# hzxie/Stereo-3D-Reconstruction

Hardware: NVIDIA B200
Metric: stereo pairs/sec Stereo2Voxel fwd (higher is better)
Workload: dtype bf16

## Files before the change

### include/s3d.h

```cpp
#ifndef S3D_H_
#define S3D_H_

#include <stdint.h>

#ifdef __cplusplus
extern "C" {
#endif

#define S3D_OK                0
#define S3D_ERR_INVALID      -1
#define S3D_ERR_CUDA         -2
#define S3D_ERR_UNSUPPORTED  -3

#define S3D_DTYPE_F32   0
#define S3D_DTYPE_BF16  1
#define S3D_DTYPE_BF16X2 2

#define S3D_ACT_NONE     0
#define S3D_ACT_RELU     1
#define S3D_ACT_LEAKY    2
#define S3D_ACT_SIGMOID  3
#define S3D_ACT_TANH     4

#define S3D_MAX_TAPS 64
// ... 33 lines not shown
                    const void* residual, void* out, void* stream);

int s3d_conv2d_halo(const void* in, const void* w, const float* bias, const void* residual, void* out, int nimg, int h, int wd,
                    int cin, int cout, int64_t osN, int64_t osH, int64_t osW, int relu, void* stream);

int s3d_pack_image(const float* img, const float* disp, float disp_scale, void* out,
                   int B, int H, int W, int Cpad, int out_dtype, void* stream);

int s3d_pack_image_u8(const uint8_t* img, const float* disp, float disp_scale, float img_scale, void* out,
                      int B, int H, int W, int Cpad, int out_dtype, void* stream);

int s3d_conv_first(const void* img, int img_u8, const float* disp, float disp_scale, const void* w, const float* bias,
                   void* out, int B, int H, int W, int cin, int cin_pad, int cout_pad, int dtype, int act,
                   float act_param, void* stream);

int s3d_conv_concat_volume(const S3dConvParams* p, const void* feat, int feat_pitch, int feat_pad, const float* bias,
                           void* out, void* stream);
int s3d_conv_concat_volume_ro(const S3dConvParams* p, const void* feat, int feat_pitch, int feat_pad, const void* w_refonce,
                              const float* bias, void* out, void* stream);
int s3d_concat_gonce_assemble(const float* maps_l, const float* maps_r, const float* edge_l, const float* edge_r,
                              const float* bias, void* out, int B, int D, int h, int w, int map_w, int out_dtype, void* stream);
int s3d_map_conv(const void* in, const void* w, float* out, int nimg, int h, int in_w, int ow, int off, int ntx, int cout,
                 int dtype, void* stream);
int s3d_cost_volume_concat(const void* feat, void* vol, int B, int h, int w, int C, int D,
                           int dtype, void* stream);
int s3d_soft_argmin(const float* cost, float* disp, int N, int D, int h, int w, float sign,
                    void* stream);


int s3d_tap_gather_soft_argmin(const float* taps, float* disp, float* disp_std_q, float* cost_out, int N, int D, int h, int w,
                               int tap_stride, float sign, void* stream);
int s3d_cls_soft_argmin(const void* x, const void* w_taps, float* disp, float* disp_std_q, int N, int D, int h, int w, int C,
                        float sign, void* stream);
int64_t s3d_conv_cls_workspace_bytes(int N, int D, int h, int w);
int s3d_conv_cls_soft_argmin(const S3dConvParams* p, const void* in, const float* bias, const void* w_taps, void* workspace,
                             float* disp, float* disp_std_q, float sign, void* stream);
int s3d_corr_soft_argmin(const void* feat, float* disp, float* disp_std_q, float* cost_out, int B, int h, int w,
                         int C, int c_real, int D, int dtype, void* stream);
int s3d_upsample_disp(const float* disp_q, float* disp, int N, int h, int w, int H, int W,
                      float scale, void* stream);
int s3d_upsample_disp_eval(const float* disp_q, float* disp, int B, int h, int w, int H, int W, float scale,
                           const float* gt, const float* thresholds, int T, float max_gt, long long* disp_stats,
                           uint8_t* lr_mask, float lr_thresh, long long* lr_stats,
                           const float* disp_std_q, float* disp_std, const float* unc_thresh, int K, long long* unc_stats,
                           void* stream);

// ... 36 lines not shown
```

### stereo_3d_reconstruction_b200/csrc/map_conv.cu

```cuda
#include <cuda.h>
#include <string.h>
#include "common.cuh"
#include "ptx.cuh"
#include "epilogue.cuh"

namespace s3d {
namespace {

constexpr int kThreads = 384;
constexpr int kTY = 16, kTX = 8;
constexpr int kMaxSlots = 6;
constexpr int kTapBytes = 8192;

struct McArgs {
  float* out;
  int nimg, h, ow, cout;
  int off;
  int ntx, ntaps, pitch;
  int patch_tx;
  int patch_bytes;
  int slots, nchunks;
  int tiles_x, tiles_per_img, total_tiles;
  uint32_t idesc;
};

struct McCtrl {
  uint64_t w_full, w_empty;
  uint64_t p_full[kMaxSlots], p_empty[kMaxSlots];
  uint64_t acc_full[2], acc_empty[2];
  uint32_t tmem_base;
};

template <int NTX, bool kSplit>
__global__ void __launch_bounds__(kThreads, 1)
map_conv_kernel(const __grid_constant__ CUtensorMap map_x, const __grid_constant__ CUtensorMap map_w, const __grid_constant__ McArgs a) {
  constexpr int kRowB = kSplit ? 128 : 64;
  constexpr int kNC = kSplit ? 64 : 128;
  constexpr uint64_t kLayout = kSplit ? 2ull : 4ull;
  static_assert(kNC * kRowB == kTapBytes, "tap bytes");
  extern __shared__ uint8_t smem_raw[];
  uint8_t* smem = reinterpret_cast<uint8_t*>((reinterpret_cast<uintptr_t>(smem_raw) + 1023) & ~uintptr_t(1023));
  uint8_t* smem_w = smem;
  uint8_t* smem_p = smem + a.ntaps * kTapBytes;
  __shared__ McCtrl ctrl;
  const int warp = threadIdx.x >> 5, lane = threadIdx.x & 31;

// ... 20 lines not shown
        for (int t0 = 0; t0 < a.ntaps; t0 += a.ntx)
          ptx::tma_load_3d(smem_w + t0 * kTapBytes, &map_w, &ctrl.w_full, 0, ch * kNC, t0);
        wphase ^= 1;
        for (int k = 0; k < my_tiles; ++k) {
          const int t = blockIdx.x + k * gridDim.x;
          const int img = t / a.tiles_per_img, r = t % a.tiles_per_img;
          const int y0 = (r / a.tiles_x) * kTY, j0 = (r % a.tiles_x) * kTX;
          ptx::mbar_wait(&ctrl.p_empty[slot], pphase ^ 1);
          ptx::mbar_arrive_expect_tx(&ctrl.p_full[slot], a.patch_tx);
          ptx::tma_load_5d(smem_p + slot * a.patch_bytes, &map_x, &ctrl.p_full[slot], 0, j0 + a.off, y0 - 1, 0, img);
          if (++slot == a.slots) { slot = 0; pphase ^= 1; }
        }
      }
    }
  } else if (warp == 1) {
    int slot = 0;  uint32_t pphase = 0, wphase = 0, aphase = 0;
    int buf = 0;
    const uint64_t hi_a = (static_cast<uint64_t>((a.pitch * kRowB) >> 4) << 32) | (1ull << 46) | (kLayout << 61);
    const uint64_t hi_b = (static_cast<uint64_t>((8 * kRowB) >> 4) << 32) | (1ull << 46) | (kLayout << 61);
    const uint32_t w_u = ptx::smem_u32(smem_w), p_u = ptx::smem_u32(smem_p);
    for (int ch = 0; ch < a.nchunks; ++ch) {
      ptx::mbar_wait(&ctrl.w_full, wphase);
      wphase ^= 1;
      for (int k = 0; k < my_tiles; ++k) {
        ptx::mbar_wait(&ctrl.acc_empty[buf], aphase ^ 1);
        ptx::mbar_wait(&ctrl.p_full[slot], pphase);
        ptx::tc_fence_after();
        const uint32_t pa = p_u + slot * a.patch_bytes, d_tmem = tmem_base + buf * kNC;
        const uint64_t ad0 = hi_a | ((pa >> 4) | (1u << 16)), bd0 = hi_b | ((w_u >> 4) | (1u << 16));
        if (ptx::elect_one()) {
#pragma unroll
          for (int t = 0; t < 3 * NTX; ++t) {
            constexpr int kPitch = kTX + NTX - 1;
            const uint64_t ad = ad0 + (uint64_t)((((t / NTX) * kPitch + (t % NTX)) * kRowB) >> 4);
            const uint64_t bd = bd0 + (uint64_t)((t * kTapBytes) >> 4);
            ptx::mma_bf16(d_tmem, ad, bd, a.idesc, t != 0);
            ptx::mma_bf16(d_tmem, ad + 2, bd + 2, a.idesc, 1u);
            if constexpr (kSplit) {
              ptx::mma_bf16(d_tmem, ad + 4, bd, a.idesc, 1u);      ptx::mma_bf16(d_tmem, ad + 6, bd + 2, a.idesc, 1u);
              ptx::mma_bf16(d_tmem, ad, bd + 4, a.idesc, 1u);      ptx::mma_bf16(d_tmem, ad + 2, bd + 6, a.idesc, 1u);
            }
          }
          ptx::tc_commit(&ctrl.p_empty[slot]);
          ptx::tc_commit(&ctrl.acc_full[buf]);
          if (k == my_tiles - 1) ptx::tc_commit(&ctrl.w_empty);
        }
        __syncwarp();
        if (++slot == a.slots) { slot = 0; pphase ^= 1; }
        if (++buf == 2) { buf = 0; aphase ^= 1; }
      }
      if (my_tiles == 0 && ptx::elect_one()) ptx::mbar_arrive(&ctrl.w_empty);
      __syncwarp();
    }
  } else if (warp >= 4) {
    const int q = warp & 3, grp = (warp - 4) >> 2;
    const int m = q * 32 + lane, yy = m >> 3, xx = m & 7;
    uint32_t aphase = 0;
    const int items = a.nchunks * my_tiles;
    for (int it = grp; it < items; it += 2) {
      const int ch = it / my_tiles, k = it % my_tiles;
      const int t = blockIdx.x + k * gridDim.x;
      const int img = t / a.tiles_per_img, r = t % a.tiles_per_img;
      const int y = (r / a.tiles_x) * kTY + yy, jt = (r % a.tiles_x) * kTX;
      float* op = a.out + (((int64_t)img * a.h + y) * a.ow + jt) * a.cout + ch * kNC + xx * 4;
      ptx::mbar_wait(&ctrl.acc_full[grp], aphase);
      ptx::tc_fence_after();
      const uint32_t taddr = tmem_base + grp * kNC + (static_cast<uint32_t>(q * 32) << 16);
#pragma unroll
      for (int half = 0; half < kNC / 64; ++half) {
        uint32_t v[4][16];
#pragma unroll
        for (int g = 0; g < 4; ++g) ptx::tmem_ld16(taddr + half * 64 + g * 16, v[g]);
        ptx::tmem_ld_wait();
        if (half == kNC / 64 - 1) {
          ptx::tc_fence_before();
          ptx::mbar_arrive(&ctrl.acc_empty[grp]);
        }
#pragma unroll
        for (int blk = 0; blk < 2; ++blk) {
          uint4 c[8];
#pragma unroll
          for (int i = 0; i < 8; ++i) {
            const uint32_t* src = &v[2 * blk + (i >> 2)][4 * (i & 3)];
            c[i] = make_uint4(src[0], src[1], src[2], src[3]);
          }
#pragma unroll
          for (int st = 4; st >= 1; st >>= 1) {
            const bool up = (lane & st) != 0;
#pragma unroll
            for (int i = 0; i < 8; ++i) {
              if (i & st) continue;
              const uint4 send = up ? c[i] : c[i | st];
              uint4 recv;
              recv.x = __shfl_xor_sync(0xffffffffu, send.x, st);  recv.y = __shfl_xor_sync(0xffffffffu, send.y, st);
              recv.z = __shfl_xor_sync(0xffffffffu, send.z, st);  recv.w = __shfl_xor_sync(0xffffffffu, send.w, st);
              if (up) c[i] = recv; else c[i | st] = recv;
            }
          }
          if (y < a.h) {
#pragma unroll
            for (int i = 0; i < 8; ++i)
              if (jt + i < a.ow) *reinterpret_cast<uint4*>(op + (int64_t)i * a.cout + half * 64 + blk * 32) = c[i];
          }
        }
      }
      aphase ^= 1;
    }
  }

  ptx::tc_fence_before();
  __syncthreads();
  if (warp == 2) {
    ptx::tc_fence_after();
    ptx::tmem_dealloc(tmem_base, 2 * kNC);
  }
}

}
}

extern "C" int s3d_map_conv(const void* in, const void* w, float* out, int nimg, int h, int in_w, int ow, int off, int ntx,
                            int cout, int dtype, void* stream) {
  using namespace s3d;
  if (!in || !w || !out) { set_error("map_conv: null argument"); return S3D_ERR_INVALID; }
  S3D_CHECK_ARG(dtype == S3D_DTYPE_BF16 || dtype == S3D_DTYPE_BF16X2, "map_conv: dtype %d (bf16 or the bf16 pair)", dtype);
  const bool split = dtype == S3D_DTYPE_BF16X2;
  const int kNC = split ? 64 : 128, kRowB = split ? 128 : 64;
  S3D_CHECK_ARG(nimg > 0 && h > 0 && ow > 0 && in_w > 0 && (ntx == 3 || ntx == 5) && cout > 0 && cout % 128 == 0,
                "map_conv: nimg=%d h=%d ow=%d in_w=%d ntx=%d cout=%d (ntx 3 or 5, cout a multiple of 128)", nimg, h, ow, in_w, ntx, cout);
  S3D_CHECK_ARG(off >= 0 && off + ow + ntx - 1 <= in_w + 8, "map_conv: output columns reach beyond the input rows");
  S3D_CHECK_ARG(((reinterpret_cast<uintptr_t>(in) | reinterpret_cast<uintptr_t>(w) | reinterpret_cast<uintptr_t>(out)) & 15) == 0,
                "map_conv: pointers must be 16-byte aligned");
  McArgs a;
  memset(&a, 0, sizeof(a));
  a.out = out;  a.nimg = nimg;  a.h = h;  a.ow = ow;  a.cout = cout;  a.off = off;
  a.ntx = ntx;  a.ntaps = 3 * ntx;  a.pitch = kTX + ntx - 1;
  a.patch_tx = (kTY + 2) * a.pitch * kRowB;
  a.patch_bytes = (a.patch_tx + 1023) / 1024 * 1024;
  a.nchunks = cout / kNC;
  a.tiles_x = ceil_div(ow, kTX);
  a.tiles_per_img = a.tiles_x * ceil_div(h, kTY);
  const int64_t total = (int64_t)nimg * a.tiles_per_img;
  S3D_CHECK_ARG(total < (1ll << 30), "map_conv: too many tiles");
  a.total_tiles = (int)total;
  a.idesc = ptx::make_instr_desc(1, 128, kNC);
  const int w_bytes = a.ntaps * kTapBytes;
  a.slots = (200 * 1024 - w_bytes) / a.patch_bytes;
  if (a.slots > kMaxSlots) a.slots = kMaxSlots;
  S3D_CHECK_ARG(a.slots >= 2, "map_conv: shared memory");
  CUtensorMap map_x, map_w;
  const CUtensorMapSwizzle sw = split ? CU_TENSOR_MAP_SWIZZLE_128B : CU_TENSOR_MAP_SWIZZLE_64B;
  const int cphys = kRowB / 2;
  cuuint32_t box[5] = {(cuuint32_t)cphys, (cuuint32_t)a.pitch, kTY + 2, 1, 1};
  cuuint32_t estr[5] = {1, 1, 1, 1, 1};
  int rc = encode_act_map(&map_x, in, 2, false, cphys, in_w, h, 1, nimg, box, estr, sw);
  if (rc != S3D_OK) return rc;
  rc = encode_weight_map(&map_w, w, 2, false, cphys, cout, a.ntaps, cphys, kNC, sw, ntx);
  if (rc != S3D_OK) return rc;
  const int smem_bytes = w_bytes + a.slots * a.patch_bytes + 1024;
  int grid = num_sms();
  if (grid > a.total_tiles) grid = a.total_tiles;
  cudaStream_t st = static_cast<cudaStream_t>(stream);
#define S3D_MC_LAUNCH(NTX_, SPLIT_)                                                                                              \
  do {                                                                                                                           \
    S3D_CUDA(cudaFuncSetAttribute(map_conv_kernel<NTX_, SPLIT_>, cudaFuncAttributeMaxDynamicSharedMemorySize, smem_bytes));       \
    map_conv_kernel<NTX_, SPLIT_><<<grid, kThreads, smem_bytes, st>>>(map_x, map_w, a);                                           \
  } while (0)
  if (ntx == 5) { if (split) S3D_MC_LAUNCH(5, true); else S3D_MC_LAUNCH(5, false); }
  else          { if (split) S3D_MC_LAUNCH(3, true); else S3D_MC_LAUNCH(3, false); }
#undef S3D_MC_LAUNCH
  S3D_LAUNCH_CHECK();
  return S3D_OK;
}
```

### stereo_3d_reconstruction_b200/layers.py

```python
import ctypes
import os
import itertools

import torch

from . import lib as _lib

PAD = 16


def pad_to(c, m=PAD):
    return (c + m - 1) // m * m


def torch_dtype(code):
    return torch.float32 if code == _lib.DTYPE_F32 else torch.bfloat16


def is_split(code):
    return code == _lib.DTYPE_BF16X2


def cmult(code):
    return 2 if code == _lib.DTYPE_BF16X2 else 1
# ... 217 lines not shown
                            if kz == 2:
                                r[5 * Ap:5 * Ap + A] -= Wr[kz, iy, dx + 1]
            taps = [[(0, dy, e + pad - 2) for dy in (-1, 0, 1) for e in es]]
            out[name + '_geom'] = (pad - 4, 5, w + 4)
            out[name] = PackedConv(rows, torch.zeros(6 * Ap), taps, (1, 1, 1), (1, 1, 1), C, 6 * Ap, _lib.ACT_NONE, 0.0,
                                   self.dtype_code, dev, ksize=(1, 3, P - (w + 4) + 1), pad=(0, 1, 0))
            dxe = -1 if name == 'left' else 1
            rows = torch.zeros(9, 4 * Ap, C)
            for iy in range(3):
                for kz in range(3):
                    e = dxe + sgn * (kz - 1)
                    ie = e + 2 if name == 'left' else e
                    r = rows[iy * 3 + ie]
                    r[0:A] -= Wr[kz, iy, dxe + 1]
                    if kz == 0:
                        r[Ap:Ap + A] += Wr[kz, iy, dxe + 1]
                    if kz == 2:
                        r[2 * Ap:2 * Ap + A] += Wr[kz, iy, dxe + 1]
            off = (pad - 2) if name == 'left' else (pad + w - D)
            taps = [[(0, dy, ie + off) for dy in (-1, 0, 1) for ie in range(3)]]
            out['edge_' + name + '_geom'] = (off, 3, D)
            out['edge_' + name] = PackedConv(rows, torch.zeros(4 * Ap), taps, (1, 1, 1), (1, 1, 1), C, 4 * Ap, _lib.ACT_NONE, 0.0,
                                             self.dtype_code, dev, ksize=(1, 3, P - D + 1), pad=(0, 1, 0))
        self._cache[key] = out
        return out

    @classmethod
    def from_conv(cls, conv, bn, act, dtype_code, device, act_param=0.0):
        w, b = _fold_bn(conv.weight, conv.bias, bn)
        if w.dim() == 4:
            w = w.unsqueeze(2)
            ks, st, pd = (1,) + tuple(conv.kernel_size), (1,) + tuple(conv.stride), (0,) + tuple(conv.padding)
        else:
            ks, st, pd = tuple(conv.kernel_size), tuple(conv.stride), tuple(conv.padding)
        cout, cin = w.shape[0], w.shape[1]
        taps, rows = [], []
        for kz, ky, kx in itertools.product(range(ks[0]), range(ks[1]), range(ks[2])):
            taps.append((kz - pd[0], ky - pd[1], kx - pd[2]))
            rows.append(w[:, :, kz, ky, kx])
        return cls(torch.stack(rows), b, [taps], st, (1, 1, 1), cin, cout, act, act_param, dtype_code, device,
                   ksize=ks, pad=pd)

    @classmethod
    def from_deconv_k4s2p1(cls, deconv, bn, act, dtype_code, device, act_param=0.0):
        assert tuple(deconv.kernel_size) == (4, 4, 4) and tuple(deconv.stride) == (2, 2, 2) and \
            tuple(deconv.padding) == (1, 1, 1) and tuple(deconv.output_padding) == (0, 0, 0)
# ... 238 lines not shown
```

### stereo_3d_reconstruction_b200/lib.py

```python
import ctypes
import os

_HERE = os.path.dirname(os.path.abspath(__file__))
LIB_PATH = os.environ.get('S3D_LIB_PATH') or os.path.join(_HERE, 'libs3d_b200.so')

S3D_MAX_TAPS = 64
DTYPE_F32, DTYPE_BF16, DTYPE_BF16X2 = 0, 1, 2
ACT_NONE, ACT_RELU, ACT_LEAKY, ACT_SIGMOID, ACT_TANH = 0, 1, 2, 3, 4


class S3dConvParams(ctypes.Structure):
    _fields_ = [
        ('N', ctypes.c_int32), ('iD', ctypes.c_int32), ('iH', ctypes.c_int32), ('iW', ctypes.c_int32),
        ('Cin', ctypes.c_int32),
        ('oD', ctypes.c_int32), ('oH', ctypes.c_int32), ('oW', ctypes.c_int32), ('Cout', ctypes.c_int32),
        ('sz', ctypes.c_int32), ('sy', ctypes.c_int32), ('sx', ctypes.c_int32),
        ('ntaps', ctypes.c_int32), ('n_classes', ctypes.c_int32),
        ('dz', ctypes.c_int8 * S3D_MAX_TAPS), ('dy', ctypes.c_int8 * S3D_MAX_TAPS),
        ('dx', ctypes.c_int8 * S3D_MAX_TAPS),
        ('osN', ctypes.c_int64), ('osD', ctypes.c_int64), ('osH', ctypes.c_int64), ('osW', ctypes.c_int64),
        ('osC', ctypes.c_int64),
        ('os_lo', ctypes.c_int64),
        ('omz', ctypes.c_int32), ('omy', ctypes.c_int32), ('omx', ctypes.c_int32),
        ('cout_store', ctypes.c_int32),
# ... 9 lines not shown


_vp, _i, _f, _i64 = ctypes.c_void_p, ctypes.c_int, ctypes.c_float, ctypes.c_int64
_CONV_SIG = [ctypes.POINTER(S3dConvParams), _vp, _vp, _vp, _vp, _vp, _vp]

SIGNATURES = {
    's3d_version': ([], ctypes.c_char_p),
    's3d_last_error': ([], ctypes.c_char_p),
    's3d_device_check': ([_i], _i),
    's3d_set_knob': ([ctypes.c_char_p, _i], _i),
    's3d_get_knob': ([ctypes.c_char_p], _i),
    's3d_conv_igemm': (_CONV_SIG, _i),
    's3d_conv_direct': (_CONV_SIG, _i),
    's3d_pack_image': ([_vp, _vp, _f, _vp, _i, _i, _i, _i, _i, _vp], _i),
    's3d_pack_image_u8': ([_vp, _vp, _f, _f, _vp, _i, _i, _i, _i, _i, _vp], _i),
    's3d_conv_first': ([_vp, _i, _vp, _f, _vp, _vp, _vp, _i, _i, _i, _i, _i, _i, _i, _i, _f, _vp], _i),
    's3d_conv_concat_volume': ([ctypes.POINTER(S3dConvParams), _vp, _i, _i, _vp, _vp, _vp], _i),
    's3d_conv_concat_volume_ro': ([ctypes.POINTER(S3dConvParams), _vp, _i, _i, _vp, _vp, _vp, _vp], _i),
    's3d_conv_cls_workspace_bytes': ([_i, _i, _i, _i], ctypes.c_int64),
    's3d_conv_cls_soft_argmin': ([ctypes.POINTER(S3dConvParams), _vp, _vp, _vp, _vp, _vp, _vp, ctypes.c_float, _vp], _i),
    's3d_conv2d_halo': ([_vp, _vp, _vp, _vp, _vp, _i, _i, _i, _i, _i, _i64, _i64, _i64, _i, _vp], _i),
    's3d_map_conv': ([_vp, _vp, _vp, _i, _i, _i, _i, _i, _i, _i, _i, _vp], _i),
    's3d_concat_gonce_assemble': ([_vp, _vp, _vp, _vp, _vp, _vp, _i, _i, _i, _i, _i, _i, _vp], _i),
    's3d_cost_volume_concat': ([_vp, _vp, _i, _i, _i, _i, _i, _i, _vp], _i),
    's3d_soft_argmin': ([_vp, _vp, _i, _i, _i, _i, _f, _vp], _i),
    's3d_tap_gather_soft_argmin': ([_vp, _vp, _vp, _vp, _i, _i, _i, _i, _i, _f, _vp], _i),
    's3d_cls_soft_argmin': ([_vp, _vp, _vp, _vp, _i, _i, _i, _i, _i, _f, _vp], _i),
    's3d_corr_soft_argmin': ([_vp, _vp, _vp, _vp, _i, _i, _i, _i, _i, _i, _i, _vp], _i),
    's3d_upsample_disp': ([_vp, _vp, _i, _i, _i, _i, _i, _f, _vp], _i),
    's3d_upsample_disp_eval': ([_vp, _vp, _i, _i, _i, _i, _i, _f,
                                _vp, ctypes.POINTER(_f), _i, _f, _vp,
                                _vp, _f, _vp,
                                _vp, _vp, ctypes.POINTER(_f), _i, _vp, _vp], _i),
    's3d_latent_to_vox': ([_vp, _vp, _i, _i, _i, _i, _i, _i, _vp], _i),
    's3d_avg_pool': ([_vp, _vp, _i, _i, _i, _i, _i, _i, _vp], _i),
    's3d_depth_to_space': ([_vp, _vp, _vp, _i, _i, _i, _i, _i, _i, _i, _vp], _i),
    's3d_split_tf32': ([_vp, _vp, _vp, _i64, _vp], _i),
    's3d_split_bf16': ([_vp, _vp, _i64, _i, _vp], _i),
    's3d_unsplit_bf16': ([_vp, _vp, _i64, _i, _vp], _i),
    's3d_fuse_views': ([_vp, _i64, _vp, _i64, _i, _vp, _i, _i, _i, _vp, ctypes.POINTER(_f), _i, _vp, _i64, _i64, _vp], _i),
    's3d_voxel_surface_workspace_bytes': ([_i, _i, _i], ctypes.c_int64),
    's3d_voxel_surface_eval': ([_vp, _vp, _i, _i, ctypes.POINTER(_f), _i, ctypes.POINTER(_i), _i, _vp, _vp, _i64, _vp], _i),
    's3d_voxel_mesh_bounds': ([_i, ctypes.POINTER(_i), ctypes.POINTER(_i)], _i),
    's3d_voxel_mesh': ([_vp, _i, _i, _f, _vp, _i, _vp, _i, _vp, _vp], _i),
    's3d_chamfer_forward': ([_vp, _vp, _vp, _vp, _vp, _vp, _i, _i, _i, _vp], _i),
    's3d_chamfer_workspace_bytes': ([_i, _i, _i], ctypes.c_int64),
# ... 63 lines not shown
```

### stereo_3d_reconstruction_b200/models.py

```python
import ctypes
import math
import os

import torch
import torch.nn as nn

from . import lib as _lib
from . import ops
from .layers import PackedConv, SplitConv, pad_to, torch_dtype, cmult, more_columns_than_pairs

A = _lib

PRECISIONS = ('bf16', 'bf16x3', 'tf32', 'tf32x3', 'fp32')


def _conv_bn2d(cin, cout, k, s, p):
    return nn.Sequential(nn.Conv2d(cin, cout, k, s, p, bias=False), nn.BatchNorm2d(cout))


def _conv_bn3d(cin, cout):
    return nn.Sequential(nn.Conv3d(cin, cout, 3, 1, 1, bias=False), nn.BatchNorm3d(cout))


class _FeatureEncoder(nn.Module):
# ... 250 lines not shown
        fuse_volume = (cfg.NETWORK.COST_VOLUME == 'concat' and (self.precision in ('bf16', 'tf32') or ro_split) and p5.cout_pad == C and
                       isinstance(p0, PackedConv) and p0.weight_ns is not None and
                       (ro_split or C * x.element_size() in (32, 64)) and
                       not _lib.KNOBS['no_concat_fuse'] and not _lib.KNOBS['no_scatter'] and
                       (sheared or more_columns_than_pairs(2 * B, h, w)))
        cm = cmult(self._dtype_code())
        if fuse_volume:
            pad, P = D, w + 2 * D
            Cp = cm * C
            featp = self._buf('featp', (2 * B, 1, h, P, Cp), dt, zero=True)
            self._conv('enc5', x, out=featp, out_view=(pad * Cp, (h * P * Cp, h * P * Cp, P * Cp, Cp), C if self._split else 0),
                       cout_store=C)
            feat = None
        else:
            feat = self._conv('enc5', x, out=self._bufo('e5', 'enc5', x))
        disp_q = self._buf('disp_q', (2 * B, h, w), torch.float32)
        std_q = self._buf('disp_std_q', (2 * B, h, w), torch.float32) if uncertainty else None
        std_kw = {} if std_q is None else {'std_out': std_q}
        if cfg.NETWORK.COST_VOLUME == 'concat':
            if fuse_volume:
                ro = ro_split or (self.precision == 'bf16' and p0.cout_pad == 64 and p0.act == _lib.ACT_RELU and
                                  not _lib.KNOBS['no_ref_once'])
                if sheared:
                    bufs = {'maps_l': self._buf('sh_ml', (B, 1, h, w + 4, 384), torch.float32),
                            'maps_r': self._buf('sh_mr', (B, 1, h, w + 4, 384), torch.float32),
                            'edge_l': self._buf('sh_el', (B, 1, h, D, 256), torch.float32),
                            'edge_r': self._buf('sh_er', (B, 1, h, D, 256), torch.float32)}
                    a = ops.conv_concat_volume_sheared(p0, featp, B, D, pad, out=self._buf('a0', (2 * B, D, h, w, cm * 64), dt), bufs=bufs)
                else:
                    a = ops.conv_concat_volume(p0, featp, B, D, pad, out=self._buf('a0', (2 * B, D, h, w, cm * p0.cout_pad), dt),
                                               ref_once=ro)
            else:
                assert feat.shape[-1] == cm * C, 'FEAT_CHANNELS must be a multiple of 16'
                vol = ops.cost_volume_concat(feat, B, D, out=self._buf('vol', (2 * B, D, h, w, 2 * cm * C), dt), split=self._split)
                a = self._conv('dres0a', vol, out=self._bufo('a0', 'dres0a', vol))
            bf = self.precision == 'bf16'
            a = self._conv('dres0b', a, out=self._bufo('a1', 'dres0b', a), dz=(B, 3, 1) if bf else None)
            y = self._conv('dres1a', a, out=self._bufo('a2', 'dres1a', a), dz=(B, 5, 2) if bf else None)
            a = self._conv('dres1b', y, residual=a, out=self._bufo('a3', 'dres1b', y), dz=(B, 7, 3) if bf else None)
            S = self._packed['cls_b'].cout_pad
            pa = self._packed['cls_a']
            if (self.precision == 'bf16' and isinstance(pa, PackedConv) and pa.weight_ns is not None and pa.cin_pad == 64 and
                    pa.cout_pad == 64 and pa.act == _lib.ACT_RELU and S == 32 and a.shape[-1] == 64 and
                    more_columns_than_pairs(2 * B, h, w) and
                    not _lib.KNOBS['no_cls_chain'] and not _lib.KNOBS['no_cls_fused'] and not _lib.KNOBS['no_scatter']):
                nb = ops.conv_cls_workspace_bytes(2 * B, D, h, w)
                ops.conv_cls_soft_argmin(pa, a, self._packed['cls_b'].weight, -1.0, out=disp_q,
                                         workspace=self._buf('cls_ws', (nb,), torch.uint8), **std_kw)
                disp, stats, lr, unc = self._upsample_disp(disp_q, H, W, disp_gt, lr_check, std_q)
                return disp, disp_q, stats, lr, unc
# ... 390 lines not shown
```

### stereo_3d_reconstruction_b200/ops.py

```python
import ctypes
import math

import torch

from . import lib as _lib


def _code(t):
    if t.dtype == torch.bfloat16:
        return _lib.DTYPE_BF16
    if t.dtype == torch.float32:
        return _lib.DTYPE_F32
    raise TypeError('unsupported dtype %s' % t.dtype)


def _code_like(t, split):
    if split:
        assert t.dtype == torch.bfloat16 and t.shape[-1] % 2 == 0
        return _lib.DTYPE_BF16X2
    return _code(t)


def _chk(*ts):
    for t in ts:
# ... 169 lines not shown
    n2, one, h, pitch, C = featp.shape
    C //= cm
    assert n2 == 2 * B and one == 1 and featp.is_contiguous() and pc.cin_pad == 2 * C and pad >= D - 1
    assert not split or ref_once, 'split (BF16X2) operands: reference-once form only'
    w = pitch - 2 * pad
    assert w > 0
    Co = cm * pc.cout_pad
    if out is None:
        out = torch.empty((2 * B, D, h, w, Co), dtype=featp.dtype, device=featp.device)
    assert out.is_contiguous() and out.shape == (2 * B, D, h, w, Co)
    p = pc.params(2 * B, D, h, w, (D * h * w * Co, h * w * Co, w * Co, Co), _code_like(out, split), pc.cout_pad)
    if ref_once:
        rc = _lib.load().s3d_conv_concat_volume_ro(ctypes.byref(p), featp.data_ptr(), pitch, pad, pc.refonce_weights(C).data_ptr(),
                                                   pc.bias.data_ptr(), out.data_ptr(), _stream())
        _lib.check(rc, 's3d_conv_concat_volume_ro')
    else:
        rc = _lib.load().s3d_conv_concat_volume(ctypes.byref(p), featp.data_ptr(), pitch, pad, pc.bias.data_ptr(), out.data_ptr(),
                                                _stream())
        _lib.check(rc, 's3d_conv_concat_volume')
    _lib.count_launch()
    return out


def conv_concat_volume_sheared(pc, featp, B, D, pad, out=None, bufs=None):
    from .layers import is_split
    _chk(featp, out)
    split = is_split(pc.dtype_code)
    cm = 2 if split else 1
    n2, one, h, pitch, C = featp.shape
    C //= cm
    assert n2 == 2 * B and one == 1 and featp.is_contiguous() and featp.dtype == torch.bfloat16
    assert pc.cin_pad == 2 * C and pc.cout_pad == 64 and pc.act == _lib.ACT_RELU and pad >= D - 1 and D >= 2
    w = pitch - 2 * pad
    g = pc.gonce_convs(C, pad, w, D)
    bufs = {} if bufs is None else bufs
    res = {}
    use_mc = C == 32 and not _lib.KNOBS['no_map_conv']
    for name, key, sl in (('left', 'maps_l', slice(0, B)), ('right', 'maps_r', slice(B, 2 * B)),
                          ('edge_left', 'edge_l', slice(0, B)), ('edge_right', 'edge_r', slice(B, 2 * B))):
        conv = g[name]
        off, ntx, ow = g[name + '_geom']
        o = bufs.get(key)
        if o is None:
            o = torch.empty((B, 1, h, ow, conv.cout_pad), dtype=torch.float32, device=featp.device)
        assert o.shape == (B, 1, h, ow, conv.cout_pad) and o.dtype == torch.float32 and o.is_contiguous()
        if use_mc:
            x = featp[sl]
            rc = _lib.load().s3d_map_conv(x.data_ptr(), conv.weight.data_ptr(), o.data_ptr(), B, h, pitch, ow, off, ntx,
                                          conv.cout_pad, pc.dtype_code, _stream())
            _lib.check(rc, 's3d_map_conv')
            _lib.count_launch()
            res[key] = o
        else:
            res[key] = conv(featp[sl], out=o)
    Co = cm * 64
    if out is None:
        out = torch.empty((2 * B, D, h, w, Co), dtype=torch.bfloat16, device=featp.device)
    assert out.is_contiguous() and out.shape == (2 * B, D, h, w, Co) and out.dtype == torch.bfloat16
    rc = _lib.load().s3d_concat_gonce_assemble(res['maps_l'].data_ptr(), res['maps_r'].data_ptr(), res['edge_l'].data_ptr(),
                                               res['edge_r'].data_ptr(), pc.bias.data_ptr(), out.data_ptr(), B, D, h, w, w + 4,
                                               _lib.DTYPE_BF16X2 if split else _lib.DTYPE_BF16, _stream())
    _lib.check(rc, 's3d_concat_gonce_assemble')
    _lib.count_launch()
    return out


def cls_soft_argmin(x, w_taps, sign=-1.0, out=None, std_out=None):
    _chk(x, w_taps, out)
    assert x.dtype == torch.bfloat16 and w_taps.dtype == torch.bfloat16 and x.dim() == 5 and x.is_contiguous()
    N, D, h, w, C = x.shape
    assert w_taps.numel() == 32 * C and w_taps.is_contiguous()
    if out is None:
        out = torch.empty((N, h, w), dtype=torch.float32, device=x.device)
    std = None if std_out is None else _std_buf(std_out, out).data_ptr()
    rc = _lib.load().s3d_cls_soft_argmin(x.data_ptr(), w_taps.data_ptr(), out.data_ptr(), std, N, D, h, w, C, float(sign),
                                         _stream())
    _lib.check(rc, 's3d_cls_soft_argmin')
    _lib.count_launch()
    return out


def conv_cls_workspace_bytes(N, D, h, w):
    return int(_lib.load().s3d_conv_cls_workspace_bytes(N, D, h, w))


# ... 276 lines not shown
```

Measured before the change: 5155.

## Fuse reference-view conv into sheared concat-volume assembly pass with tcgen05 MMA

For the bf16 non-split C=32 case, the map convolutions now compute only the target-view half of the channels (192 instead of 384/256). A new persistent kernel recomputes the reference-view 3x3 conv on tensor cores into TMEM and adds the shifted target maps, edge terms and bias per disparity plane before writing the volume. This replaces the separate assemble kernel and halves the fp32 map intermediates written and read. The cost is a larger, more complex warp-specialised kernel that needs a partial-chunk path in map_conv for cout that is a multiple of 64.

```diff
diff --git a/include/s3d.h b/include/s3d.h
--- a/include/s3d.h
+++ b/include/s3d.h
@@ -79,6 +79,9 @@
                               const float* bias, void* out, int B, int D, int h, int w, int map_w, int out_dtype, void* stream);
 int s3d_map_conv(const void* in, const void* w, float* out, int nimg, int h, int in_w, int ow, int off, int ntx, int cout,
                  int dtype, void* stream);
+int s3d_concat_sheared_pass(const void* featp, const void* w_ref, const float* maps_l, const float* maps_r, const float* edge_l,
+                            const float* edge_r, const float* bias, void* out, int B, int D, int h, int w, int pitch, int pad,
+                            void* stream);
 int s3d_cost_volume_concat(const void* feat, void* vol, int B, int h, int w, int C, int D,
                            int dtype, void* stream);
 int s3d_soft_argmin(const float* cost, float* disp, int N, int D, int h, int w, float sign,
diff --git a/stereo_3d_reconstruction_b200/csrc/map_conv.cu b/stereo_3d_reconstruction_b200/csrc/map_conv.cu
--- a/stereo_3d_reconstruction_b200/csrc/map_conv.cu
+++ b/stereo_3d_reconstruction_b200/csrc/map_conv.cu
@@ -20,8 +20,9 @@
   int patch_tx;
   int patch_bytes;
   int slots, nchunks;
+  int last_nc;
   int tiles_x, tiles_per_img, total_tiles;
-  uint32_t idesc;
+  uint32_t idesc, idesc_last;
 };
 
 struct McCtrl {
@@ -88,6 +89,7 @@
     for (int ch = 0; ch < a.nchunks; ++ch) {
       ptx::mbar_wait(&ctrl.w_full, wphase);
       wphase ^= 1;
+      const uint32_t idesc = ch == a.nchunks - 1 ? a.idesc_last : a.idesc;
       for (int k = 0; k < my_tiles; ++k) {
         ptx::mbar_wait(&ctrl.acc_empty[buf], aphase ^ 1);
         ptx::mbar_wait(&ctrl.p_full[slot], pphase);
@@ -100,11 +102,11 @@
             constexpr int kPitch = kTX + NTX - 1;
             const uint64_t ad = ad0 + (uint64_t)((((t / NTX) * kPitch + (t % NTX)) * kRowB) >> 4);
             const uint64_t bd = bd0 + (uint64_t)((t * kTapBytes) >> 4);
-            ptx::mma_bf16(d_tmem, ad, bd, a.idesc, t != 0);
-            ptx::mma_bf16(d_tmem, ad + 2, bd + 2, a.idesc, 1u);
+            ptx::mma_bf16(d_tmem, ad, bd, idesc, t != 0);
+            ptx::mma_bf16(d_tmem, ad + 2, bd + 2, idesc, 1u);
             if constexpr (kSplit) {
-              ptx::mma_bf16(d_tmem, ad + 4, bd, a.idesc, 1u);      ptx::mma_bf16(d_tmem, ad + 6, bd + 2, a.idesc, 1u);
-              ptx::mma_bf16(d_tmem, ad, bd + 4, a.idesc, 1u);      ptx::mma_bf16(d_tmem, ad + 2, bd + 6, a.idesc, 1u);
+              ptx::mma_bf16(d_tmem, ad + 4, bd, idesc, 1u);      ptx::mma_bf16(d_tmem, ad + 6, bd + 2, idesc, 1u);
+              ptx::mma_bf16(d_tmem, ad, bd + 4, idesc, 1u);      ptx::mma_bf16(d_tmem, ad + 2, bd + 6, idesc, 1u);
             }
           }
           ptx::tc_commit(&ctrl.p_empty[slot]);
@@ -132,13 +134,15 @@
       ptx::mbar_wait(&ctrl.acc_full[grp], aphase);
       ptx::tc_fence_after();
       const uint32_t taddr = tmem_base + grp * kNC + (static_cast<uint32_t>(q * 32) << 16);
+      const int nhalf = (ch == a.nchunks - 1 ? a.last_nc : kNC) / 64;
 #pragma unroll
       for (int half = 0; half < kNC / 64; ++half) {
+        if (half == nhalf) break;
         uint32_t v[4][16];
 #pragma unroll
         for (int g = 0; g < 4; ++g) ptx::tmem_ld16(taddr + half * 64 + g * 16, v[g]);
         ptx::tmem_ld_wait();
-        if (half == kNC / 64 - 1) {
+        if (half == nhalf - 1) {
           ptx::tc_fence_before();
           ptx::mbar_arrive(&ctrl.acc_empty[grp]);
         }
@@ -182,6 +186,255 @@
   }
 }
 
+
+constexpr int kPassN = 192;
+constexpr int kPassTapBytes = kPassN * 64;
+constexpr int kPassTaps = 9;
+constexpr int kPassGroups = 2;
+constexpr int kPassThreads = 128 + 128 * kPassGroups;
+constexpr int kPassBuf = 256;
+constexpr int kPassMaps = 3 * 64;
+
+struct PassArgs {
+  const float *maps_l, *maps_r, *edge_l, *edge_r, *bias;
+  __nv_bfloat16* out;
+  int B, D, h, w, mw;
+  int off;
+  int patch_tx, patch_bytes, slots;
+  int tiles_x, tiles_per_img, total_tiles;
+  uint32_t idesc;
+};
+
+struct PassCtrl {
+  uint64_t w_full;
+  uint64_t p_full[kMaxSlots], p_empty[kMaxSlots];
+  uint64_t acc_full[2], acc_empty[2];
+  uint32_t tmem_base;
+};
+
+__device__ __forceinline__ void pass_ld_octets(uint32_t taddr, float (&r)[8][8], int lane) {
+  uint32_t v[4][16];
+#pragma unroll
+  for (int g = 0; g < 4; ++g) ptx::tmem_ld16(taddr + g * 16, v[g]);
+  ptx::tmem_ld_wait();
+#pragma unroll
+  for (int part = 0; part < 2; ++part) {
+    uint4 c[8];
+#pragma unroll
+    for (int i = 0; i < 8; ++i) {
+      const uint32_t* src = &v[i >> 1][(i & 1) * 8 + part * 4];
+      c[i] = make_uint4(src[0], src[1], src[2], src[3]);
+    }
+#pragma unroll
+    for (int st = 4; st >= 1; st >>= 1) {
+      const bool up = (lane & st) != 0;
+#pragma unroll
+      for (int i = 0; i < 8; ++i) {
+        if (i & st) continue;
+        const uint4 send = up ? c[i] : c[i | st];
+        uint4 recv;
+        recv.x = __shfl_xor_sync(0xffffffffu, send.x, st);  recv.y = __shfl_xor_sync(0xffffffffu, send.y, st);
+        recv.z = __shfl_xor_sync(0xffffffffu, send.z, st);  recv.w = __shfl_xor_sync(0xffffffffu, send.w, st);
+        if (up) c[i] = recv; else c[i | st] = recv;
+      }
+    }
+#pragma unroll
+    for (int i = 0; i < 8; ++i) {
+      r[i][part * 4 + 0] = __uint_as_float(c[i].x);  r[i][part * 4 + 1] = __uint_as_float(c[i].y);
+      r[i][part * 4 + 2] = __uint_as_float(c[i].z);  r[i][part * 4 + 3] = __uint_as_float(c[i].w);
+    }
+  }
+}
+
+__device__ __forceinline__ void pass_add8(float (&v)[8], const float* __restrict__ p) {
+  const float4 a = __ldg(reinterpret_cast<const float4*>(p)), b = __ldg(reinterpret_cast<const float4*>(p) + 1);
+  v[0] += a.x;  v[1] += a.y;  v[2] += a.z;  v[3] += a.w;  v[4] += b.x;  v[5] += b.y;  v[6] += b.z;  v[7] += b.w;
+}
+
+template <int kBorder>
+__device__ __forceinline__ void pass_plane(const PassArgs& a, int d, const float (&base)[8][8], const float (&border)[8][8],
+                                           const float* __restrict__ gm, const float* __restrict__ em, __nv_bfloat16* op,
+                                           bool left_ref, int x0, int xe) {
+  constexpr int kB = kBorder ? 1 : 8;
+#pragma unroll
+  for (int i0 = 0; i0 < 8; i0 += kB) {
+    float4 gl[kB][2], hl[kB][2];
+    bool in[kB];
+#pragma unroll
+    for (int i = 0; i < kB; ++i) {
+      const int x = x0 + i0 + i;
+      const int col = (left_ref ? x - d : x + d) + 2;
+      in[i] = x < a.w && col >= 0 && col < a.mw;
+      const float4* g = reinterpret_cast<const float4*>(gm + (int64_t)(in[i] ? col : 0) * kPassMaps);
+      gl[i][0] = make_float4(0.f, 0.f, 0.f, 0.f);  gl[i][1] = gl[i][0];  hl[i][0] = gl[i][0];  hl[i][1] = gl[i][0];
+      if (in[i]) {
+        gl[i][0] = __ldg(g);  gl[i][1] = __ldg(g + 1);
+        if constexpr (kBorder != 0) { hl[i][0] = __ldg(g + kBorder * 16);  hl[i][1] = __ldg(g + kBorder * 16 + 1); }
+      }
+    }
+#pragma unroll
+    for (int i = 0; i < kB; ++i) {
+      const int x = x0 + i0 + i;
+      if (x >= a.w) continue;
+      float v[8];
+#pragma unroll
+      for (int j = 0; j < 8; ++j) v[j] = base[i0 + i][j];
+      if (in[i]) {
+        v[0] += gl[i][0].x;  v[1] += gl[i][0].y;  v[2] += gl[i][0].z;  v[3] += gl[i][0].w;
+        v[4] += gl[i][1].x;  v[5] += gl[i][1].y;  v[6] += gl[i][1].z;  v[7] += gl[i][1].w;
+      }
+      if constexpr (kBorder != 0) {
+#pragma unroll
+        for (int j = 0; j < 8; ++j) v[j] += border[i0 + i][j];
+        if (in[i]) {
+          v[0] += hl[i][0].x;  v[1] += hl[i][0].y;  v[2] += hl[i][0].z;  v[3] += hl[i][0].w;
+          v[4] += hl[i][1].x;  v[5] += hl[i][1].y;  v[6] += hl[i][1].z;  v[7] += hl[i][1].w;
+        }
+      }
+      if (x == xe) {
+        const float* e = em + (int64_t)(left_ref ? a.D - 1 - d : d) * kPassMaps;
+        pass_add8(v, e);
+        if constexpr (kBorder != 0) pass_add8(v, e + kBorder * 64);
+      }
+      uint32_t o[4];
+#pragma unroll
+      for (int k = 0; k < 4; ++k) {
+        __nv_bfloat162 t = __floats2bfloat162_rn(fmax_nan(v[2 * k], 0.f), fmax_nan(v[2 * k + 1], 0.f));
+        o[k] = *reinterpret_cast<uint32_t*>(&t);
+      }
+      __stcs(reinterpret_cast<uint4*>(op + (int64_t)(i0 + i) * 64), make_uint4(o[0], o[1], o[2], o[3]));
+    }
+  }
+}
+
+__global__ void __launch_bounds__(kPassThreads, 1)
+concat_sheared_pass_kernel(const __grid_constant__ CUtensorMap map_x, const __grid_constant__ CUtensorMap map_w,
+                           const __grid_constant__ PassArgs a) {
+  constexpr int kPitch = kTX + 2;
+  extern __shared__ uint8_t smem_raw[];
+  uint8_t* smem = reinterpret_cast<uint8_t*>((reinterpret_cast<uintptr_t>(smem_raw) + 1023) & ~uintptr_t(1023));
+  uint8_t* smem_w = smem;
+  uint8_t* smem_p = smem + kPassTaps * kPassTapBytes;
+  __shared__ PassCtrl ctrl;
+  const int warp = threadIdx.x >> 5, lane = threadIdx.x & 31;
+
+  if (warp == 0 && lane == 0) { ptx::prefetch_tensormap(&map_x);  ptx::prefetch_tensormap(&map_w); }
+  if (warp == 1 && lane == 0) {
+    ptx::mbar_init(&ctrl.w_full, 1);
+    for (int s = 0; s < kMaxSlots; ++s) { ptx::mbar_init(&ctrl.p_full[s], 1);  ptx::mbar_init(&ctrl.p_empty[s], 1); }
+    for (int b = 0; b < 2; ++b) { ptx::mbar_init(&ctrl.acc_full[b], 1);  ptx::mbar_init(&ctrl.acc_empty[b], 128 * kPassGroups); }
+    ptx::fence_barrier_init();
+  }
+  if (warp == 2) ptx::tmem_alloc(&ctrl.tmem_base, 2 * kPassBuf);
+  ptx::tc_fence_before();
+  __syncthreads();
+  ptx::tc_fence_after();
+  const uint32_t tmem_base = ctrl.tmem_base;
+  const int my_tiles = a.total_tiles > (int)blockIdx.x ? (a.total_tiles - (int)blockIdx.x + (int)gridDim.x - 1) / (int)gridDim.x : 0;
+
+  if (warp == 0) {
+    if (lane == 0) {
+      ptx::mbar_arrive_expect_tx(&ctrl.w_full, kPassTaps * kPassTapBytes);
+      for (int t0 = 0; t0 < kPassTaps; t0 += 3)
+        ptx::tma_load_3d(smem_w + t0 * kPassTapBytes, &map_w, &ctrl.w_full, 0, 0, t0);
+      int slot = 0;  uint32_t pphase = 0;
+      for (int k = 0; k < my_tiles; ++k) {
+        const int t = blockIdx.x + k * gridDim.x;
+        const int img = t / a.tiles_per_img, r = t % a.tiles_per_img;
+        const int y0 = (r / a.tiles_x) * kTY, j0 = (r % a.tiles_x) * kTX;
+        ptx::mbar_wait(&ctrl.p_empty[slot], pphase ^ 1);
+        ptx::mbar_arrive_expect_tx(&ctrl.p_full[slot], a.patch_tx);
+        ptx::tma_load_5d(smem_p + slot * a.patch_bytes, &map_x, &ctrl.p_full[slot], 0, j0 + a.off, y0 - 1, 0, img);
+        if (++slot == a.slots) { slot = 0; pphase ^= 1; }
+      }
+    }
+  } else if (warp == 1) {
+    int slot = 0;  uint32_t pphase = 0;
+    const uint64_t hi_a = (static_cast<uint64_t>((kPitch * 64) >> 4) << 32) | (1ull << 46) | (4ull << 61);
+    const uint64_t hi_b = (static_cast<uint64_t>((8 * 64) >> 4) << 32) | (1ull << 46) | (4ull << 61);
+    const uint32_t w_u = ptx::smem_u32(smem_w), p_u = ptx::smem_u32(smem_p);
+    ptx::mbar_wait(&ctrl.w_full, 0);
+    for (int k = 0; k < my_tiles; ++k) {
+      const int buf = k & 1;
+      ptx::mbar_wait(&ctrl.acc_empty[buf], ((k >> 1) & 1) ^ 1);
+      ptx::mbar_wait(&ctrl.p_full[slot], pphase);
+      ptx::tc_fence_after();
+      const uint32_t pa = p_u + slot * a.patch_bytes, d_tmem = tmem_base + buf * kPassBuf;
+      const uint64_t ad0 = hi_a | ((pa >> 4) | (1u << 16)), bd0 = hi_b | ((w_u >> 4) | (1u << 16));
+      if (ptx::elect_one()) {
+#pragma unroll
+        for (int t = 0; t < kPassTaps; ++t) {
+          const uint64_t ad = ad0 + (uint64_t)((((t / 3) * kPitch + (t % 3)) * 64) >> 4);
+          const uint64_t bd = bd0 + (uint64_t)((t * kPassTapBytes) >> 4);
+          ptx::mma_bf16(d_tmem, ad, bd, a.idesc, t != 0);
+          ptx::mma_bf16(d_tmem, ad + 2, bd + 2, a.idesc, 1u);
+        }
+        ptx::tc_commit(&ctrl.p_empty[slot]);
+        ptx::tc_commit(&ctrl.acc_full[buf]);
+      }
+      __syncwarp();
+      if (++slot == a.slots) { slot = 0; pphase ^= 1; }
+    }
+  } else if (warp >= 4) {
+    const int q = warp & 3, grp = (warp - 4) >> 2;
+    const int yy = (q * 32 + lane) >> 3, xx = lane & 7;
+    float bias[8];
+#pragma unroll
+    for (int j = 0; j < 8; ++j) bias[j] = __ldg(a.bias + xx * 8 + j);
+    const int64_t plane = (int64_t)a.h * a.w * 64;
+    for (int k = 0; k < my_tiles; ++k) {
+      const int buf = k & 1;
+      const int t = blockIdx.x + k * gridDim.x;
+      const int img = t / a.tiles_per_img, r = t % a.tiles_per_img;
+      const int y = (r / a.tiles_x) * kTY + yy, x0 = (r % a.tiles_x) * kTX;
+      const bool left_ref = img < a.B;
+      const int b = left_ref ? img : img - a.B;
+      const int xe = left_ref ? a.w - 1 : 0;
+      const bool row = y < a.h;
+      const float* gm = (left_ref ? a.maps_r : a.maps_l) + ((int64_t)b * a.h + y) * a.mw * kPassMaps + xx * 8;
+      const float* em = (left_ref ? a.edge_r : a.edge_l) + ((int64_t)b * a.h + y) * a.D * kPassMaps + xx * 8;
+      __nv_bfloat16* op = a.out + (((int64_t)img * a.D * a.h + y) * a.w + x0) * 64 + xx * 8;
+      if (row) {
+        const int c0 = left_ref ? max(x0 + 3 - a.D, 0) : x0 + 2, c1 = min(left_ref ? x0 + kTX + 2 : x0 + kTX + 1 + a.D, a.mw);
+        for (int c = c0 + xx; c < c1; c += 8) {
+          const float* p = gm - xx * 8 + (int64_t)c * kPassMaps;
+          asm volatile("prefetch.global.L2 [%0];" ::"l"(p));
+          asm volatile("prefetch.global.L2 [%0];" ::"l"(p + 32));
+        }
+      }
+      ptx::mbar_wait(&ctrl.acc_full[buf], (k >> 1) & 1);
+      ptx::tc_fence_after();
+      const uint32_t taddr = tmem_base + buf * kPassBuf + (static_cast<uint32_t>(q * 32) << 16);
+      float base[8][8], border[8][8];
+      pass_ld_octets(taddr, base, lane);
+#pragma unroll
+      for (int i = 0; i < 8; ++i)
+#pragma unroll
+        for (int j = 0; j < 8; ++j) base[i][j] = bias[j] + base[i][j];
+      if (grp == 0) {
+        pass_ld_octets(taddr + 64, border, lane);
+        if (row) pass_plane<1>(a, 0, base, border, gm, em, op, left_ref, x0, xe);
+      }
+      if (grp == (a.D - 1) % kPassGroups) {
+        pass_ld_octets(taddr + 128, border, lane);
+        if (row) pass_plane<2>(a, a.D - 1, base, border, gm, em, op + (a.D - 1) * plane, left_ref, x0, xe);
+      }
+      ptx::tc_fence_before();
+      ptx::mbar_arrive(&ctrl.acc_empty[buf]);
+      if (row)
+        for (int d = grp == 0 ? kPassGroups : grp; d < a.D - 1; d += kPassGroups)
+          pass_plane<0>(a, d, base, border, gm, em, op + d * plane, left_ref, x0, xe);
+    }
+  }
+
+  ptx::tc_fence_before();
+  __syncthreads();
+  if (warp == 2) {
+    ptx::tc_fence_after();
+    ptx::tmem_dealloc(tmem_base, 2 * kPassBuf);
+  }
+}
+
 }
 }
 
@@ -192,8 +445,8 @@
   S3D_CHECK_ARG(dtype == S3D_DTYPE_BF16 || dtype == S3D_DTYPE_BF16X2, "map_conv: dtype %d (bf16 or the bf16 pair)", dtype);
   const bool split = dtype == S3D_DTYPE_BF16X2;
   const int kNC = split ? 64 : 128, kRowB = split ? 128 : 64;
-  S3D_CHECK_ARG(nimg > 0 && h > 0 && ow > 0 && in_w > 0 && (ntx == 3 || ntx == 5) && cout > 0 && cout % 128 == 0,
-                "map_conv: nimg=%d h=%d ow=%d in_w=%d ntx=%d cout=%d (ntx 3 or 5, cout a multiple of 128)", nimg, h, ow, in_w, ntx, cout);
+  S3D_CHECK_ARG(nimg > 0 && h > 0 && ow > 0 && in_w > 0 && (ntx == 3 || ntx == 5) && cout > 0 && cout % 64 == 0,
+                "map_conv: nimg=%d h=%d ow=%d in_w=%d ntx=%d cout=%d (ntx 3 or 5, cout a multiple of 64)", nimg, h, ow, in_w, ntx, cout);
   S3D_CHECK_ARG(off >= 0 && off + ow + ntx - 1 <= in_w + 8, "map_conv: output columns reach beyond the input rows");
   S3D_CHECK_ARG(((reinterpret_cast<uintptr_t>(in) | reinterpret_cast<uintptr_t>(w) | reinterpret_cast<uintptr_t>(out)) & 15) == 0,
                 "map_conv: pointers must be 16-byte aligned");
@@ -203,13 +456,15 @@
   a.ntx = ntx;  a.ntaps = 3 * ntx;  a.pitch = kTX + ntx - 1;
   a.patch_tx = (kTY + 2) * a.pitch * kRowB;
   a.patch_bytes = (a.patch_tx + 1023) / 1024 * 1024;
-  a.nchunks = cout / kNC;
+  a.nchunks = ceil_div(cout, kNC);
+  a.last_nc = cout - (a.nchunks - 1) * kNC;
   a.tiles_x = ceil_div(ow, kTX);
   a.tiles_per_img = a.tiles_x * ceil_div(h, kTY);
   const int64_t total = (int64_t)nimg * a.tiles_per_img;
   S3D_CHECK_ARG(total < (1ll << 30), "map_conv: too many tiles");
   a.total_tiles = (int)total;
   a.idesc = ptx::make_instr_desc(1, 128, kNC);
+  a.idesc_last = ptx::make_instr_desc(1, 128, a.last_nc);
   const int w_bytes = a.ntaps * kTapBytes;
   a.slots = (200 * 1024 - w_bytes) / a.patch_bytes;
   if (a.slots > kMaxSlots) a.slots = kMaxSlots;
@@ -238,3 +493,47 @@
   S3D_LAUNCH_CHECK();
   return S3D_OK;
 }
+
+extern "C" int s3d_concat_sheared_pass(const void* featp, const void* w_ref, const float* maps_l, const float* maps_r,
+                                       const float* edge_l, const float* edge_r, const float* bias, void* out, int B, int D, int h,
+                                       int w, int pitch, int pad, void* stream) {
+  using namespace s3d;
+  if (!featp || !w_ref || !maps_l || !maps_r || !edge_l || !edge_r || !bias || !out) {
+    set_error("concat_sheared_pass: null argument");
+    return S3D_ERR_INVALID;
+  }
+  S3D_CHECK_ARG(B > 0 && D >= 2 && h > 0 && w > 0 && pad >= 1 && pitch == w + 2 * pad,
+                "concat_sheared_pass: B=%d D=%d h=%d w=%d pitch=%d pad=%d (needs D >= 2, pad >= 1, pitch = w + 2 pad)", B, D, h, w, pitch, pad);
+  S3D_CHECK_ARG(((reinterpret_cast<uintptr_t>(featp) | reinterpret_cast<uintptr_t>(w_ref) | reinterpret_cast<uintptr_t>(maps_l) |
+                  reinterpret_cast<uintptr_t>(maps_r) | reinterpret_cast<uintptr_t>(edge_l) | reinterpret_cast<uintptr_t>(edge_r) |
+                  reinterpret_cast<uintptr_t>(bias) | reinterpret_cast<uintptr_t>(out)) & 15) == 0,
+                "concat_sheared_pass: pointers must be 16-byte aligned");
+  PassArgs a;
+  memset(&a, 0, sizeof(a));
+  a.maps_l = maps_l;  a.maps_r = maps_r;  a.edge_l = edge_l;  a.edge_r = edge_r;  a.bias = bias;
+  a.out = static_cast<__nv_bfloat16*>(out);
+  a.B = B;  a.D = D;  a.h = h;  a.w = w;  a.mw = w + 4;  a.off = pad - 1;
+  a.patch_tx = (kTY + 2) * (kTX + 2) * 64;
+  a.patch_bytes = (a.patch_tx + 1023) / 1024 * 1024;
+  a.tiles_x = ceil_div(w, kTX);
+  a.tiles_per_img = a.tiles_x * ceil_div(h, kTY);
+  const int64_t total = (int64_t)2 * B * a.tiles_per_img;
+  S3D_CHECK_ARG(total < (1ll << 30), "concat_sheared_pass: too many tiles");
+  a.total_tiles = (int)total;
+  a.idesc = ptx::make_instr_desc(1, 128, kPassN);
+  a.slots = 4;
+  CUtensorMap map_x, map_w;
+  cuuint32_t box[5] = {32, kTX + 2, kTY + 2, 1, 1};
+  cuuint32_t estr[5] = {1, 1, 1, 1, 1};
+  int rc = encode_act_map(&map_x, featp, 2, false, 32, pitch, h, 1, 2 * B, box, estr, CU_TENSOR_MAP_SWIZZLE_64B);
+  if (rc != S3D_OK) return rc;
+  rc = encode_weight_map(&map_w, w_ref, 2, false, 32, kPassN, kPassTaps, 32, kPassN, CU_TENSOR_MAP_SWIZZLE_64B, 3);
+  if (rc != S3D_OK) return rc;
+  const int smem_bytes = kPassTaps * kPassTapBytes + a.slots * a.patch_bytes + 1024;
+  int grid = num_sms();
+  if (grid > a.total_tiles) grid = a.total_tiles;
+  S3D_CUDA(cudaFuncSetAttribute(concat_sheared_pass_kernel, cudaFuncAttributeMaxDynamicSharedMemorySize, smem_bytes));
+  concat_sheared_pass_kernel<<<grid, kPassThreads, smem_bytes, static_cast<cudaStream_t>(stream)>>>(map_x, map_w, a);
+  S3D_LAUNCH_CHECK();
+  return S3D_OK;
+}
diff --git a/stereo_3d_reconstruction_b200/layers.py b/stereo_3d_reconstruction_b200/layers.py
--- a/stereo_3d_reconstruction_b200/layers.py
+++ b/stereo_3d_reconstruction_b200/layers.py
@@ -263,6 +263,13 @@
             out['edge_' + name + '_geom'] = (off, 3, D)
             out['edge_' + name] = PackedConv(rows, torch.zeros(4 * Ap), taps, (1, 1, 1), (1, 1, 1), C, 4 * Ap, _lib.ACT_NONE, 0.0,
                                              self.dtype_code, dev, ksize=(1, 3, P - D + 1), pad=(0, 1, 0))
+        if self.dtype_code == _lib.DTYPE_BF16:
+            for name in ('left', 'right'):
+                ci = out[name].weight.shape[-1]
+                out[name + '_tgt'] = out[name].weight.view(15, 6 * Ap, ci)[:, 3 * Ap:].contiguous()
+                out['edge_' + name + '_tgt'] = out['edge_' + name].weight.view(9, 4 * Ap, ci)[:, :3 * Ap].contiguous()
+            ci = out['left'].weight.shape[-1]
+            out['pass'] = out['left'].weight.view(3, 5, 6 * Ap, ci)[:, 1:4, :3 * Ap].reshape(9, 3 * Ap, ci).contiguous()
         self._cache[key] = out
         return out
 
diff --git a/stereo_3d_reconstruction_b200/lib.py b/stereo_3d_reconstruction_b200/lib.py
--- a/stereo_3d_reconstruction_b200/lib.py
+++ b/stereo_3d_reconstruction_b200/lib.py
@@ -55,6 +55,7 @@
     's3d_conv2d_halo': ([_vp, _vp, _vp, _vp, _vp, _i, _i, _i, _i, _i, _i64, _i64, _i64, _i, _vp], _i),
     's3d_map_conv': ([_vp, _vp, _vp, _i, _i, _i, _i, _i, _i, _i, _i, _vp], _i),
     's3d_concat_gonce_assemble': ([_vp, _vp, _vp, _vp, _vp, _vp, _i, _i, _i, _i, _i, _i, _vp], _i),
+    's3d_concat_sheared_pass': ([_vp, _vp, _vp, _vp, _vp, _vp, _vp, _vp, _i, _i, _i, _i, _i, _i, _vp], _i),
     's3d_cost_volume_concat': ([_vp, _vp, _i, _i, _i, _i, _i, _i, _vp], _i),
     's3d_soft_argmin': ([_vp, _vp, _i, _i, _i, _i, _f, _vp], _i),
     's3d_tap_gather_soft_argmin': ([_vp, _vp, _vp, _vp, _i, _i, _i, _i, _i, _f, _vp], _i),
diff --git a/stereo_3d_reconstruction_b200/models.py b/stereo_3d_reconstruction_b200/models.py
--- a/stereo_3d_reconstruction_b200/models.py
+++ b/stereo_3d_reconstruction_b200/models.py
@@ -296,10 +296,11 @@
                 ro = ro_split or (self.precision == 'bf16' and p0.cout_pad == 64 and p0.act == _lib.ACT_RELU and
                                   not _lib.KNOBS['no_ref_once'])
                 if sheared:
-                    bufs = {'maps_l': self._buf('sh_ml', (B, 1, h, w + 4, 384), torch.float32),
-                            'maps_r': self._buf('sh_mr', (B, 1, h, w + 4, 384), torch.float32),
-                            'edge_l': self._buf('sh_el', (B, 1, h, D, 256), torch.float32),
-                            'edge_r': self._buf('sh_er', (B, 1, h, D, 256), torch.float32)}
+                    nm, ne = ops.sheared_map_channels(self._split, C)
+                    bufs = {'maps_l': self._buf('sh_ml', (B, 1, h, w + 4, nm), torch.float32),
+                            'maps_r': self._buf('sh_mr', (B, 1, h, w + 4, nm), torch.float32),
+                            'edge_l': self._buf('sh_el', (B, 1, h, D, ne), torch.float32),
+                            'edge_r': self._buf('sh_er', (B, 1, h, D, ne), torch.float32)}
                     a = ops.conv_concat_volume_sheared(p0, featp, B, D, pad, out=self._buf('a0', (2 * B, D, h, w, cm * 64), dt), bufs=bufs)
                 else:
                     a = ops.conv_concat_volume(p0, featp, B, D, pad, out=self._buf('a0', (2 * B, D, h, w, cm * p0.cout_pad), dt),
diff --git a/stereo_3d_reconstruction_b200/ops.py b/stereo_3d_reconstruction_b200/ops.py
--- a/stereo_3d_reconstruction_b200/ops.py
+++ b/stereo_3d_reconstruction_b200/ops.py
@@ -215,6 +215,14 @@
     return out
 
 
+def sheared_pass_applies(split, C):
+    return C == 32 and not split and not _lib.KNOBS['no_map_conv']
+
+
+def sheared_map_channels(split, C):
+    return (192, 192) if sheared_pass_applies(split, C) else (384, 256)
+
+
 def conv_concat_volume_sheared(pc, featp, B, D, pad, out=None, bufs=None):
     from .layers import is_split
     _chk(featp, out)
@@ -229,18 +237,21 @@
     bufs = {} if bufs is None else bufs
     res = {}
     use_mc = C == 32 and not _lib.KNOBS['no_map_conv']
+    use_pass = sheared_pass_applies(split, C)
     for name, key, sl in (('left', 'maps_l', slice(0, B)), ('right', 'maps_r', slice(B, 2 * B)),
                           ('edge_left', 'edge_l', slice(0, B)), ('edge_right', 'edge_r', slice(B, 2 * B))):
         conv = g[name]
         off, ntx, ow = g[name + '_geom']
+        cout = g[name + '_tgt'].shape[1] if use_pass else conv.cout_pad
         o = bufs.get(key)
         if o is None:
-            o = torch.empty((B, 1, h, ow, conv.cout_pad), dtype=torch.float32, device=featp.device)
-        assert o.shape == (B, 1, h, ow, conv.cout_pad) and o.dtype == torch.float32 and o.is_contiguous()
+            o = torch.empty((B, 1, h, ow, cout), dtype=torch.float32, device=featp.device)
+        assert o.shape == (B, 1, h, ow, cout) and o.dtype == torch.float32 and o.is_contiguous()
         if use_mc:
             x = featp[sl]
-            rc = _lib.load().s3d_map_conv(x.data_ptr(), conv.weight.data_ptr(), o.data_ptr(), B, h, pitch, ow, off, ntx,
-                                          conv.cout_pad, pc.dtype_code, _stream())
+            wt = g[name + '_tgt'] if use_pass else conv.weight
+            rc = _lib.load().s3d_map_conv(x.data_ptr(), wt.data_ptr(), o.data_ptr(), B, h, pitch, ow, off, ntx, cout,
+                                          pc.dtype_code, _stream())
             _lib.check(rc, 's3d_map_conv')
             _lib.count_launch()
             res[key] = o
@@ -250,10 +261,16 @@
     if out is None:
         out = torch.empty((2 * B, D, h, w, Co), dtype=torch.bfloat16, device=featp.device)
     assert out.is_contiguous() and out.shape == (2 * B, D, h, w, Co) and out.dtype == torch.bfloat16
-    rc = _lib.load().s3d_concat_gonce_assemble(res['maps_l'].data_ptr(), res['maps_r'].data_ptr(), res['edge_l'].data_ptr(),
-                                               res['edge_r'].data_ptr(), pc.bias.data_ptr(), out.data_ptr(), B, D, h, w, w + 4,
-                                               _lib.DTYPE_BF16X2 if split else _lib.DTYPE_BF16, _stream())
-    _lib.check(rc, 's3d_concat_gonce_assemble')
+    if use_pass:
+        rc = _lib.load().s3d_concat_sheared_pass(featp.data_ptr(), g['pass'].data_ptr(), res['maps_l'].data_ptr(),
+                                                 res['maps_r'].data_ptr(), res['edge_l'].data_ptr(), res['edge_r'].data_ptr(),
+                                                 pc.bias.data_ptr(), out.data_ptr(), B, D, h, w, pitch, pad, _stream())
+        _lib.check(rc, 's3d_concat_sheared_pass')
+    else:
+        rc = _lib.load().s3d_concat_gonce_assemble(res['maps_l'].data_ptr(), res['maps_r'].data_ptr(), res['edge_l'].data_ptr(),
+                                                   res['edge_r'].data_ptr(), pc.bias.data_ptr(), out.data_ptr(), B, D, h, w, w + 4,
+                                                   _lib.DTYPE_BF16X2 if split else _lib.DTYPE_BF16, _stream())
+        _lib.check(rc, 's3d_concat_gonce_assemble')
     _lib.count_launch()
     return out
 
```

Result: slower. 4998 (median of 6 runs) (-3.0%).
